# mayataka/idocp

Hardware: AMD Instinct MI355X
Metric: SQP iterations/sec (whole node) (higher is better)
Workload: dtype f64; 1 GPU; ANYmal OCPSolver N=100 T=5.05 FP64, trotting contact sequence (1 lift + 9 impulse events, 120 stages incl. impulse / aux / lift stages, switching constraints; BASELINE.json configs[2]); batch=1024 independent OCP instances per GPU, replicas across GPUs; horizon=100, batch_per_gpu=1024, parallelism=replicas x1

## Files before the change

idocp_amd/csrc/dev_rnea_tangent.hpp:

```cpp
#ifndef IDOCP_DEV_RNEA_TANGENT_HPP_
#define IDOCP_DEV_RNEA_TANGENT_HPP_

#include <hip/hip_runtime.h>

#include "dev_rbd.hpp"
#include "ocp_device.hpp"

namespace idocp_dev {

namespace rt {
struct V3 { double x, y, z; };
__device__ __forceinline__ V3 v3(double x, double y, double z) { V3 r; r.x = x; r.y = y; r.z = z; return r; }
__device__ __forceinline__ V3 ld3(const double* p) { return v3(p[0], p[1], p[2]); }
__device__ __forceinline__ void st3(double* p, V3 a) { p[0] = a.x; p[1] = a.y; p[2] = a.z; }
__device__ __forceinline__ V3 operator+(V3 a, V3 b) { return v3(a.x + b.x, a.y + b.y, a.z + b.z); }
__device__ __forceinline__ V3 operator-(V3 a, V3 b) { return v3(a.x - b.x, a.y - b.y, a.z - b.z); }
__device__ __forceinline__ V3 operator*(double s, V3 a) { return v3(s * a.x, s * a.y, s * a.z); }
__device__ __forceinline__ V3 cross(V3 a, V3 b) { return v3(a.y * b.z - a.z * b.y, a.z * b.x - a.x * b.z, a.x * b.y - a.y * b.x); }
__device__ __forceinline__ double dot(V3 a, V3 b) { return a.x * b.x + a.y * b.y + a.z * b.z; }
__device__ __forceinline__ V3 mul(const double* R, V3 a) {
  return v3(R[0] * a.x + R[1] * a.y + R[2] * a.z, R[3] * a.x + R[4] * a.y + R[5] * a.z, R[6] * a.x + R[7] * a.y + R[8] * a.z);
}
__device__ __forceinline__ V3 mulT(const double* R, V3 a) {
  return v3(R[0] * a.x + R[3] * a.y + R[6] * a.z, R[1] * a.x + R[4] * a.y + R[7] * a.z, R[2] * a.x + R[5] * a.y + R[8] * a.z);
// ... 130 lines not shown
  double* didc; int ldd;
  double* mm;
  double* jm; int ldj;
  double* idc;
};

template <typename D>
__device__ __forceinline__ void rneaSetup(const DevModel* __restrict__ m, const OcpProblem* __restrict__ P, const OcpNode* __restrict__ nd,
                                          int tid, double* sc) {
  using S = RneaScratch<D>;
  using namespace rt;
  constexpr int NL = D::NL, LJ = D::LJ, NJL = NL * LJ;
  if (tid >= 128 && tid < 128 + NJL) {
    const int t = tid - 128, ji = 1 + t;
    double* jr = sc + S::JOINTS + t * S::JREC;
    st3(jr + S::J_U, ld3(m->axis[ji])); st3(jr + S::J_P, ld3(m->p[ji]));
    jr[S::J_MASS] = m->mass[ji]; st3(jr + S::J_MC, ld3(m->mc[ji]));
#pragma unroll
    for (int e = 0; e < 6; ++e) jr[S::J_IO + e] = m->Io[ji][e];
  } else if (tid >= 192 && tid < 192 + NL) {
    const int leg = tid - 192;
    double* fr = sc + S::FEET + leg * S::FREC;
#pragma unroll
    for (int e = 0; e < 9; ++e) fr[S::F_RC + e] = P->contact_R[leg][e];
    st3(fr + S::F_PC, ld3(P->contact_p[leg]));
    fr[S::F_ACT] = nd->active[leg] ? 1.0 : 0.0;
    fr[S::F_ROW] = (double)nd->row_of[leg];
  } else if (tid == 192 + NL) {
    double* br = sc + S::BASE;
    br[S::B_MASS] = m->mass[0]; st3(br + S::B_MC, ld3(m->mc[0]));
#pragma unroll
    for (int e = 0; e < 6; ++e) br[S::B_IO + e] = m->Io[0][e];
  }
}

template <typename D, int NT>
struct RneaNominalCopy {
  using S = RneaScratch<D>;
  typedef double d2 __attribute__((ext_vector_type(2)));
  static constexpr int PER = (S::C_ALL + NT - 1) / NT;
  d2 r[PER];
  __device__ __forceinline__ void fetch(const double* __restrict__ nom, int tid) {
#pragma unroll
    for (int t = 0; t < PER; ++t) {
      const int c = tid + NT * t;
      r[t] = *reinterpret_cast<const d2*>(nom + 2 * (c < S::C_ALL ? c : 0));
    }
  }
  __device__ __forceinline__ void store(int tid, double* sc, double* idc) const {
#pragma unroll
    for (int t = 0; t < PER; ++t) {
      const int c = tid + NT * t;
      if (c < S::C_BN) *reinterpret_cast<d2*>(sc + S::pieceDst(c)) = r[t];
      else if (c < S::C_ALL) *reinterpret_cast<d2*>(idc + 2 * (c - S::C_BN)) = r[t];
    }
  }
};

template <typename D, bool XYY = false, bool IMPULSE = false>
__device__ __forceinline__ void rneaTangentItem(double gz, double wv, int item, double* sc, const RneaOut& out) {
  using S = RneaScratch<D>;
  using namespace rt;
  constexpr int LJ = D::LJ, NV = D::NV;
  const int leg = item / S::IPL, j0 = item - leg * S::IPL;
  const bool base_seed = j0 < 18;
  const int kind = base_seed ? j0 / 6 : (j0 - 18) / LJ;
  const int k = base_seed ? j0 - 6 * kind : 6 + leg * LJ + (j0 - 18 - LJ * kind);
  double* __restrict__ colp = (kind < 2) ? out.didc + (long)out.ldd * (kind * NV + k) : out.mm + NV * k;
  double* __restrict__ colc = (kind < 2) ? colp + NV : out.jm + (long)out.ldj * k;
  const double* br = sc + S::BASE;
  auto e3 = [](int i) { return v3(i == 0 ? 1.0 : 0.0, i == 1 ? 1.0 : 0.0, i == 2 ? 1.0 : 0.0); };
  const V3 zero = v3(0, 0, 0);
  V3 dz = (kind == 0 && k >= 3 && k < 6) ? cross(ld3(br + S::B_Z), e3(k - 3)) : zero;
  V3 dv = (kind == 1 && k < 3) ? e3(k) : zero, dw = (kind == 1 && k >= 3 && k < 6) ? e3(k - 3) : zero;
  V3 dbl = ((kind == 2 && k < 3) ? e3(k) : zero) - gz * dz, dbw = (kind == 2 && k >= 3 && k < 6) ? e3(k - 3) : zero;
  if (leg == 0 && base_seed) {
    V3 dhl, dhn, df, dn;
    const V3 mc = ld3(br + S::B_MC);
    inertia(br[S::B_MASS], mc, br + S::B_IO, dbl, dbw, df, dn);
    double* o = sc + S::BOWN + 6 * j0;
    if constexpr (IMPULSE) {
      st3(o, df); st3(o + 3, dn);
    } else {
      const V3 w0 = ld3(br + S::B_W), v0 = ld3(br + S::B_V), hl0 = ld3(br + S::B_HL), hn0 = ld3(br + S::B_HN);
      inertia(br[S::B_MASS], mc, br + S::B_IO, dv, dw, dhl, dhn);
      st3(o, df + cross(dw, hl0) + cross(w0, dhl));
      st3(o + 3, dn + cross(dw, hn0) + cross(w0, dhn) + cross(dv, hl0) + cross(v0, dhl));
    }
  }
  double tau[LJ];
#pragma unroll
  for (int j = 0; j < LJ; ++j) tau[j] = 0.0;
  V3 baseFl = zero, baseFn = zero;
  const double* jleg = sc + S::JOINTS + leg * LJ * S::JREC;
  forEachLegJointUnrolled<XYY, true, LJ>([&](auto tag, auto jc) {
    constexpr int AX = decltype(tag)::value, j = decltype(jc)::value;
    const int dof = 6 + leg * LJ + j;
    const double* jr = jleg + j * S::JREC;
    const bool mine = (k == dof);
    const double sq = (mine && kind == 0) ? 1.0 : 0.0, sv = (mine && kind == 1) ? 1.0 : 0.0, sa = (mine && kind == 2) ? 1.0 : 0.0;
    const JointFrame<AX> F(jr, S::J_R, S::J_U);
    {
      const V3 p = ld3(jr + S::J_P);
      const V3 wj = ld3(jr + S::J_W), vj = ld3(jr + S::J_VC);
      const V3 dwc = F.mulT(dw) - F.crossUk(ld3(jr + S::J_WC), sq);
      const V3 dvc = F.mulT(dv + cross(dw, p)) - F.crossUk(vj, sq);
      const V3 dbwc = F.mulT(dbw) - F.crossUk(ld3(jr + S::J_BWC), sq);
      const V3 dblc = F.mulT(dbl + cross(dbw, p)) - F.crossUk(ld3(jr + S::J_BLC), sq);
      dz = F.mulT(dz) - F.crossUk(ld3(jr + S::J_ZC), sq);
      dw = dwc + F.timesU(sv); dv = dvc;
      if constexpr (IMPULSE) {
        dbw = dbwc + F.timesU(sa); dbl = dblc;
      } else if constexpr (AX < 0) {
        const V3 vJ = ld3(jr + S::J_VJ), dvJ = F.timesU(sv);
        dbw = dbwc + F.timesU(sa) + cross(dw, vJ) + cross(wj, dvJ);
        dbl = dblc + cross(dv, vJ) + cross(vj, dvJ);
      } else {
        const double qd = jr[S::J_VJ + (AX < 0 ? 0 : AX)];
        dbw = dbwc + F.timesU(sa) + F.crossKU(dw, qd) + F.crossKU(wj, sv);
        dbl = dblc + F.crossKU(dv, qd) + F.crossKU(vj, sv);
      }
    }
    pin(dw); pin(dv); pin(dbw); pin(dbl); pin(dz);
    phaseFence();
    V3 Fl, Fn;
    {
      if constexpr (IMPULSE) {
        inertia(jr[S::J_MASS], ld3(jr + S::J_MC), jr + S::J_IO, dbl, dbw, Fl, Fn);
      } else {
        V3 dhl, dhn;
        {
          const V3 mc = ld3(jr + S::J_MC);
          inertia(jr[S::J_MASS], mc, jr + S::J_IO, dv, dw, dhl, dhn);
          inertia(jr[S::J_MASS], mc, jr + S::J_IO, dbl, dbw, Fl, Fn);
        }
        pin(dhl); pin(dhn); pin(Fl); pin(Fn);
        phaseFence();
        const V3 wj = ld3(jr + S::J_W), vj = ld3(jr + S::J_VC), hl = ld3(jr + S::J_HL), hn = ld3(jr + S::J_HN);
        Fl = Fl + cross(dw, hl) + cross(wj, dhl);
        Fn = Fn + cross(dw, hn) + cross(wj, dhn) + cross(dv, hl) + cross(vj, dhl);
      }
    }
    pin(Fl); pin(Fn);
    phaseFence();
    auto hop = [&](auto jjc) {
      constexpr int jj = decltype(jjc)::value;
      const double* jq = jleg + jj * S::JREC;
      const LegFrame<XYY, jj> G(jq, S::J_R, S::J_U);
      tau[jj] += G.dotU(Fn);
      if constexpr (jj == j) {
        Fl = Fl + G.crossUk(ld3(jq + S::J_FL), sq);
        Fn = Fn + G.crossUk(ld3(jq + S::J_FN), sq);
      }
      const V3 Rf = G.mul(Fl);
      Fn = G.mul(Fn) + cross(ld3(jq + S::J_P), Rf);
      Fl = Rf;
    };
    downFrom<j>(hop);
    baseFl = baseFl + Fl; baseFn = baseFn + Fn;
    pin(baseFl); pin(baseFn);
#pragma unroll
    for (int t = 0; t <= j; ++t) pin(tau[t]);
  });
  phaseFence();
  const double* fr = sc + S::FEET + leg * S::FREC;
  if (fr[S::F_ACT] != 0.0) {
    const double* Rc = fr + S::F_RC;
    const V3 pc = ld3(fr + S::F_PC);
    const V3 dal = dbl + gz * dz;
    const V3 dfv = XYY ? dv + cross(dw, pc) : mulT(Rc, dv + cross(dw, pc));
    if constexpr (IMPULSE) {
      st3(colc + (int)fr[S::F_ROW], dfv);
    } else {
      const V3 dfw = XYY ? dw : mulT(Rc, dw), dfa = XYY ? dal + cross(dbw, pc) : mulT(Rc, dal + cross(dbw, pc));
      const V3 dc = dfa + cross(ld3(fr + S::F_FW), dfv) + cross(ld3(fr + S::F_FV), dfw) + wv * dfv;
      st3(colc + (int)fr[S::F_ROW], dc);
    }
  }
#pragma unroll
  for (int j = 0; j < LJ; ++j) colp[6 + leg * LJ + j] = tau[j];
  double* o = sc + S::BT + 6 * item;
  st3(o, baseFl); st3(o + 3, baseFn);
}

template <typename D, bool XYY = false>
__device__ __forceinline__ void rneaTangentItemUndo(double gz, double wv, int item, double* sc, const RneaOut& out) {
  using S = RneaScratch<D>;
  using namespace rt;
  constexpr int LJ = D::LJ, NV = D::NV;
  const int leg = item / S::IPL, j0 = item - leg * S::IPL;
  const bool base_seed = j0 < 18;
  const int kind = base_seed ? j0 / 6 : (j0 - 18) / LJ;
  const int k = base_seed ? j0 - 6 * kind : 6 + leg * LJ + (j0 - 18 - LJ * kind);
  double* __restrict__ colp = (kind < 2) ? out.didc + (long)out.ldd * (kind * NV + k) : out.mm + NV * k;
  double* __restrict__ colc = (kind < 2) ? colp + NV : out.jm + (long)out.ldj * k;
  const double* br = sc + S::BASE;
  auto e3 = [](int i) { return v3(i == 0 ? 1.0 : 0.0, i == 1 ? 1.0 : 0.0, i == 2 ? 1.0 : 0.0); };
  const V3 zero = v3(0, 0, 0);
  V3 dz = (kind == 0 && k >= 3 && k < 6) ? cross(ld3(br + S::B_Z), e3(k - 3)) : zero;
  V3 dv = (kind == 1 && k < 3) ? e3(k) : zero, dw = (kind == 1 && k >= 3 && k < 6) ? e3(k - 3) : zero;
  V3 dbl = ((kind == 2 && k < 3) ? e3(k) : zero) - gz * dz, dbw = (kind == 2 && k >= 3 && k < 6) ? e3(k - 3) : zero;
  if (leg == 0 && base_seed) {
    V3 dhl, dhn, df, dn;
    const V3 mc = ld3(br + S::B_MC), w0 = ld3(br + S::B_W), v0 = ld3(br + S::B_V), hl0 = ld3(br + S::B_HL), hn0 = ld3(br + S::B_HN);
    inertia(br[S::B_MASS], mc, br + S::B_IO, dv, dw, dhl, dhn);
    inertia(br[S::B_MASS], mc, br + S::B_IO, dbl, dbw, df, dn);
    double* o = sc + S::BOWN + 6 * j0;
    st3(o, df + cross(dw, hl0) + cross(w0, dhl));
    st3(o + 3, dn + cross(dw, hn0) + cross(w0, dhn) + cross(dv, hl0) + cross(v0, dhl));
  }
  forEachLegJoint<XYY, true, LJ>([&](auto tag, int j) {
    constexpr int AX = decltype(tag)::value;
    const int dof = 6 + leg * LJ + j;
    const double* jr = sc + S::JOINTS + (leg * LJ + j) * S::JREC;
    const bool mine = (k == dof);
    const double sq = (mine && kind == 0) ? 1.0 : 0.0, sv = (mine && kind == 1) ? 1.0 : 0.0, sa = (mine && kind == 2) ? 1.0 : 0.0;
    const JointFrame<AX> F(jr, S::J_R, S::J_U);
    const V3 p = ld3(jr + S::J_P);
    const double qd = AX < 0 ? 0.0 : jr[S::J_VJ + (AX < 0 ? 0 : AX)];
    const V3 dwc = F.mulT(dw) - F.crossUk(ld3(jr + S::J_WC), sq);
    const V3 dvc = F.mulT(dv + cross(dw, p)) - F.crossUk(ld3(jr + S::J_VC), sq);
    const V3 dbwc = F.mulT(dbw) - F.crossUk(ld3(jr + S::J_BWC), sq);
    const V3 dblc = F.mulT(dbl + cross(dbw, p)) - F.crossUk(ld3(jr + S::J_BLC), sq);
    dz = F.mulT(dz) - F.crossUk(ld3(jr + S::J_ZC), sq);
    dw = dwc + F.timesU(sv); dv = dvc;
    if constexpr (AX < 0) {
      const V3 vJ = ld3(jr + S::J_VJ), dvJ = F.timesU(sv);
      dbw = dbwc + F.timesU(sa) + cross(dw, vJ) + cross(ld3(jr + S::J_W), dvJ);
      dbl = dblc + cross(dv, vJ) + cross(ld3(jr + S::J_VC), dvJ);
    } else {
      dbw = dbwc + F.timesU(sa) + F.crossKU(dw, qd) + F.crossKU(ld3(jr + S::J_W), sv);
      dbl = dblc + F.crossKU(dv, qd) + F.crossKU(ld3(jr + S::J_VC), sv);
    }
  });
  const double* fr = sc + S::FEET + leg * S::FREC;
  if (fr[S::F_ACT] != 0.0) {
    const double* Rc = fr + S::F_RC;
    const V3 pc = ld3(fr + S::F_PC);
    const V3 dal = dbl + gz * dz;
    const V3 dfv = XYY ? dv + cross(dw, pc) : mulT(Rc, dv + cross(dw, pc)), dfw = XYY ? dw : mulT(Rc, dw),
             dfa = XYY ? dal + cross(dbw, pc) : mulT(Rc, dal + cross(dbw, pc));
    const V3 dc = dfa + cross(ld3(fr + S::F_FW), dfv) + cross(ld3(fr + S::F_FV), dfw) + wv * dfv;
    st3(colc + (int)fr[S::F_ROW], dc);
  }
  V3 dFl = zero, dFn = zero;
  forEachLegJoint<XYY, false, LJ>([&](auto tag, int j) {
    constexpr int AX = decltype(tag)::value;
    const int dof = 6 + leg * LJ + j;
    const double* jr = sc + S::JOINTS + (leg * LJ + j) * S::JREC;
    const bool mine = (k == dof);
    const double sq = (mine && kind == 0) ? 1.0 : 0.0, sv = (mine && kind == 1) ? 1.0 : 0.0, sa = (mine && kind == 2) ? 1.0 : 0.0;
    const JointFrame<AX> F(jr, S::J_R, S::J_U);
    const V3 p = ld3(jr + S::J_P), mc = ld3(jr + S::J_MC);
    const V3 wj = ld3(jr + S::J_W), vj = ld3(jr + S::J_VC), hl = ld3(jr + S::J_HL), hn = ld3(jr + S::J_HN);
    V3 dhl, dhn, df, dn;
    inertia(jr[S::J_MASS], mc, jr + S::J_IO, dv, dw, dhl, dhn);
    inertia(jr[S::J_MASS], mc, jr + S::J_IO, dbl, dbw, df, dn);
    dFl = dFl + df + cross(dw, hl) + cross(wj, dhl);
    dFn = dFn + dn + cross(dw, hn) + cross(wj, dhn) + cross(dv, hl) + cross(vj, dhl);
    colp[dof] = F.dotU(dFn);
    const V3 dRf = F.mul(dFl + F.crossUk(ld3(jr + S::J_FL), sq));
    dFn = F.mul(dFn + F.crossUk(ld3(jr + S::J_FN), sq)) + cross(p, dRf);
    dFl = dRf;
    if (j > 0) {
      V3 dbwc, dblc;
// ... 168 lines not shown
```

idocp_amd/csrc/ocp_condense_kernel.hip:

```cpp
#include <hip/hip_runtime.h>

#include <cstdlib>

#include "dev_dense.hpp"
#include "dev_lie.hpp"
#include "dev_rnea_tangent.hpp"
#include "ocp_device.hpp"
#include "ocp_launch.hpp"

namespace idocp_dev {

#ifdef IDOCP_K5_TILES16
#define K5_TILE_PAIR mfmaTilePairTN
#else
#define K5_TILE_PAIR mfmaTilePairTN4
#endif

__device__ __forceinline__ double ocpLimit(const OcpProblem* __restrict__ P, int comp, int r) {
  switch (comp) {
    case 0: return P->q_min[r];
    case 1: return P->q_max[r];
    case 2: return -P->v_max[r];
    case 3: return P->v_max[r];
    case 4: return -P->u_max[r];
    case 8: return P->a_min[r];
    case 9: return P->a_max[r];
    default: return P->u_max[r];
  }
}
__device__ __forceinline__ bool ocpRowValid(const OcpProblem* __restrict__ P, int comp, int level, bool impulse) {
  if (impulse) return comp == 6 && P->use_impulse_friction_cone != 0;
  if (comp < 2) return P->use_q_limits && level >= 2;
  if (comp < 4) return P->use_v_limits && level >= 1;
  if (comp < 6) return P->use_u_limits != 0;
  if (comp == 8) return P->use_a_lower != 0;
  if (comp == 9) return P->use_a_upper != 0;
  return comp == 6 && P->use_friction_cone != 0;
}

template <typename D, int SFP = D::NF>
struct CondenseSmem {
  using L = OcpLayout<D>;
  static constexpr int NV = D::NV, NX = D::NX, NF = SFP, NVF = D::NV + SFP + (((D::NV + SFP) % 8 == 0) ? 2 : 0), NU = D::NU;
  static constexpr bool SEP_MINV = SFP <= 6;
  static constexpr int DIDC = 0, MM = DIDC + NVF * (NX + 1), JM = MM + NV * NV,
                       IDC = JM + ((NF * NV > NVF * NV - NV * NV) ? NF * NV : NVF * NV - NV * NV),
                       MJ = IDC + 32,
                       MJD = MJ + NVF * NVF,
                       QFF = (MJD + NVF * (NX + 1) > MJ + RneaScratch<D>::TOTAL) ? MJD + NVF * (NX + 1) : MJ + RneaScratch<D>::TOTAL, TMP = QFF + NF * NF,
                       QAFQV = DIDC, QAFU = MM, ERR = MJ;
  static constexpr int SOLS = TMP, SOLN = SOLS + L::SOL, SLK = SOLN + L::SOL, DUL = SLK + L::CON, TMP_EARLY = DUL + L::CON - TMP;
  static constexpr int BL = TMP, SM = BL + NF * NV, TMP_LATE = SM + NF * NF - TMP;
  static constexpr int VEC = TMP + (TMP_EARLY > TMP_LATE ? TMP_EARLY : TMP_LATE);
  static_assert(NVF * NV <= IDC - MM, "Qafu_full must fit in the M / J blocks");
  static_assert(512 <= NVF * NVF, "ERR (two accumulators per thread in the MERIT variant) aliases MJ");
  static constexpr int LQ = VEC, LV = LQ + NV, LA = LV + NV, LF = LA + NV, LU = LF + NF, LUP = LU + NU, FQ = LUP + 6, FV = FQ + NV,
                       LAF = FV + NV, TLA = LAF + 32, QAA = TLA + 32,
                       BM = QAA + NV,
                       LIEB = BM + 32, JQ = LIEB + L::Z_JQ, QDIFF = LIEB + L::Z_QDIFF, FQQ = LIEB + L::Z_FQQ, FQ6 = LIEB + L::Z_FQ6,
                       FQQI = LIEB + L::Z_FQQI, FQQP = LIEB + L::Z_FQQP, FQQPI = LIEB + L::Z_FQQPI,
                       HQD = LIEB + 196, HVD = HQD + NV, HUD = HVD + NV, QB6 = HUD + NU,
                       MINV = SEP_MINV ? QB6 + 36 + 2 : MM,
                       WSM = QB6 + 36 + 2 + (SEP_MINV ? NV * NV : 0),
                       TOTAL = WSM + (SEP_MINV ? 0 : NF * NF);
  static_assert(SOLS % 2 == 0 && LIEB % 2 == 0 && IDC % 2 == 0 && MJ % 2 == 0, "16-byte pieces");
};

__device__ __forceinline__ void blockLdsBarrier() {
  __builtin_amdgcn_fence(__ATOMIC_RELEASE, "workgroup", "local");
  __builtin_amdgcn_s_barrier();
  __builtin_amdgcn_fence(__ATOMIC_ACQUIRE, "workgroup", "local");
}

template <typename D, bool RESIDUAL, int DIMF, bool BWD = false, bool MERIT = false, bool XYY = false, bool EVENTS = false>
__global__ __launch_bounds__(256, 4) void ocp_condense_kernel(OcpBuffers B, const double* __restrict__ q0, const double* __restrict__ v0 = nullptr,
                                                              const int* __restrict__ plist = nullptr, int nlist = 0) {
  using L = OcpLayout<D>;
  using S = CondenseSmem<D, (DIMF > 0) ? DIMF : (DIMF == 0 ? D::NF / 2 : D::NF)>;
  constexpr int NV = D::NV, NQ = D::NQ, NX = D::NX, NF = D::NF, NVF = D::NVF, NU = D::NU, NC = D::NC;
  constexpr int SF = (DIMF > 0) ? DIMF : (DIMF == 0 ? NF / 2 : NF), SVF = S::NVF, RVF = NV + SF;
  extern __shared__ __attribute__((aligned(16))) double sm[];
  __shared__ int s_ok, s_c1, s_ba, s_gt, s_m;
  const OcpProblem* __restrict__ P = B.prob;
  const int M = B.M;
  int tid = threadIdx.x;
  tid = (((tid >> 6) + (int)(blockIdx.x & 3)) & 3) * 64 + (tid & 63);
  constexpr int nt = 256;
  const int per = plist ? nlist : M;
  auto stage = [&](const long unit) {
  const long b = unit / per;
  const int pos = plist ? plist[unit - b * per] : (int)(unit - b * per);
  const OcpNode* __restrict__ nd = B.nodes + pos;
  const bool terminal = (pos == M - 1);
  if (BWD && terminal) {
    if (MERIT && threadIdx.x < 2) B.merit_stage[(b * B.NS + nd->slot) * 4 + threadIdx.x] = 0.0;
    return;
  }
  const bool last = BWD && P->has_terminal && (pos == M - 2);
  constexpr bool PLAIN = (DIMF >= 0) && !EVENTS;
  const bool impulse = PLAIN ? false : (nd->kind == 1);
  if (BWD && impulse) return;
  const int sw_dimi = PLAIN ? 0 : nd->sw_dimi;
  int c_act[NC], c_row[NC];
#pragma unroll
  for (int c = 0; c < NC; ++c) { c_act[c] = nd->active[c]; c_row[c] = nd->row_of[c]; }
  const int i = nd->level;
  const double dt = nd->dt;
  const double dtq = nd->dtq;
  const int dimf = (DIMF >= 0) ? DIMF : nd->dimf, dimvf = NV + dimf;
  const int dimfd = (DIMF == 0) ? 1 : dimf;
  const long rec = b * B.NS + nd->slot;
  const double* __restrict__ s_g = B.sol + rec * L::SOL;
  const double* __restrict__ sn_g = B.sol + (b * B.NS + (terminal ? nd->slot : nd->next)) * L::SOL;
  const double* s = &sm[S::SOLS];
  const double* sn = &sm[S::SOLN];
  const double* q = s + L::S_Q;
  const double* __restrict__ qref = B.q_ref + (long)pos * NQ;
  const long su = rec;
#ifdef IDOCP_K5_STAMPS
  const bool stamp = (!RESIDUAL) && tid == 0 && unit == (long)(gridDim.x / 2 + 7) && B.prof != nullptr && DIMF == B.prof_dimf;
#define STAMP(k) do { if (stamp) B.prof[k] = wall_clock64(); } while (0)
  const bool stampw = (!RESIDUAL) && (tid & 63) == 0 && unit == (long)(gridDim.x / 2 + 7) && B.prof != nullptr && DIMF == B.prof_dimf;
#define STAMPW(k) do { if (stampw) B.prof[32 + 8 * (tid >> 6) + (k)] = wall_clock64(); } while (0)
#else
#define STAMP(k) do { } while (0)
#define STAMPW(k) do { } while (0)
#endif
  STAMP(0);
  double* kk = B.kkt + rec * L::KKT;
  double* ee = B.exp + rec * L::EXP;
  const double* __restrict__ w_q = impulse ? P->qi_weight : P->q_weight;
  const double* __restrict__ w_v = impulse ? P->vi_weight : P->v_weight;
  const double* __restrict__ w_a = impulse ? P->dvi_weight : P->a_weight;

  using RS = RneaScratch<D>;
  using RI = RneaItems<D>;
  static_assert(S::QFF - S::MJ >= RS::TOTAL, "the RNEA scratch lives in MJ .. MJD (dead until stage 3)");
  static_assert(S::MJ % 2 == 0 && S::IDC % 2 == 0, "16-byte pieces of the nominal record");
  static_assert(RI::NQV <= 64 && RI::NA <= 64, "one wavefront per item list");
  constexpr int NPRE = (2 * L::SOL + 2 * L::CON + nt - 1) / nt;
  static_assert(S::SOLN == S::SOLS + L::SOL && S::SLK == S::SOLN + L::SOL && S::DUL == S::SLK + L::CON, "the fetched records are contiguous in LDS");
  const int wave = tid >> 6, lane = tid & 63;
  double* const sc = &sm[S::MJ];
  RneaOut out;
  out.didc = &sm[S::DIDC]; out.ldd = SVF; out.mm = &sm[S::MM]; out.jm = &sm[S::JM]; out.ldj = SF; out.idc = &sm[S::IDC];
  {
    double pre[NPRE], prez[7];
    RneaNominalCopy<D, nt> nomc;
    const bool has_nom = !terminal;
    if (has_nom) nomc.fetch(B.nom + rec * L::NOM, tid);
#pragma unroll
    for (int t = 0; t < NPRE; ++t) {
      const int e = tid + nt * t;
      const double* src = e < L::SOL ? s_g + e : (e < 2 * L::SOL ? sn_g + (e - L::SOL) : (e < 2 * L::SOL + L::CON ? B.slack + su * L::CON + (e - 2 * L::SOL)
                                                                         : B.dual + su * L::CON + (e < 2 * L::SOL + 2 * L::CON ? e - 2 * L::SOL - L::CON : 0)));
      pre[t] = *src;
    }
    {
      const double* __restrict__ zz = B.lie + rec * L::LIE;
      if (tid < 36) { prez[0] = zz[L::Z_JQ + tid]; prez[1] = zz[L::Z_FQQ + tid]; prez[2] = zz[L::Z_FQQI + tid]; prez[3] = zz[L::Z_FQQP + tid]; prez[4] = zz[L::Z_FQQPI + tid]; }
      if (tid >= 64 && tid < 70) { prez[5] = zz[L::Z_QDIFF + tid - 64]; prez[6] = zz[L::Z_FQ6 + tid - 64]; }
    }
    STAMP(3);
    if (tid == 0) { s_ok = 1; s_c1 = 0; s_ba = 0; s_gt = 0; s_m = 0; }
    if (!terminal) {
      for (int e = tid; e < S::IDC - S::DIDC; e += nt) sm[S::DIDC + e] = 0.0;
      rneaSetup<D>(B.model, P, nd, tid, sc);
      nomc.store(tid, sc, &sm[S::IDC]);
    }
    for (int e = tid; e < SF * SF; e += nt) sm[S::QFF + e] = 0.0;
#pragma unroll
    for (int t = 0; t < NPRE; ++t) {
      const int e = tid + nt * t;
      if (e < 2 * L::SOL + 2 * L::CON) sm[S::SOLS + e] = pre[t];
    }
    if (tid < 36) { sm[S::JQ + tid] = prez[0]; sm[S::FQQ + tid] = prez[1]; sm[S::FQQI + tid] = prez[2]; sm[S::FQQP + tid] = prez[3]; sm[S::FQQPI + tid] = prez[4]; }
    if (tid >= 64 && tid < 70) { sm[S::QDIFF + tid - 64] = prez[5]; sm[S::FQ6 + tid - 64] = prez[6]; }
    STAMP(4);
  }
  blockLdsBarrier();
  STAMP(1);

  const double vref_on = nd->vref_on;
  const double v_ref0 = vref_on * P->v_ref[0];
  if (terminal) {
    if (tid < NV) {
      const int r = tid;
      double lq, lv;
      if (r < 6) {
        lq = 0.0;
        for (int m2 = 0; m2 < 6; ++m2) lq += sm[S::JQ + m2 + 6 * r] * P->qf_weight[m2] * sm[S::QDIFF + m2];
        double t1 = 0.0;
        for (int m2 = 0; m2 < 6; ++m2) t1 += sm[S::FQQP + m2 + 6 * r] * s[L::S_LMD + m2];
        lq += t1;
      } else {
        lq = P->qf_weight[r] * (q[r + 1] - qref[r + 1]) - s[L::S_LMD + r];
      }
      lv = P->vf_weight[r] * (s[L::S_V + r] - (r == 0 ? v_ref0 : vref_on * P->v_ref[r])) - s[L::S_GMM + r];
      if (B.ext) lq += B.ext[rec * L::EXT + L::X_LQ + r];
      if (MERIT) {
        const double qd = r < 6 ? sm[S::QDIFF + r] : q[r + 1] - qref[r + 1], dvr = s[L::S_V + r] - (r == 0 ? v_ref0 : vref_on * P->v_ref[r]);
        sm[S::ERR + tid] = 0.5 * (P->qf_weight[r] * qd * qd + P->vf_weight[r] * dvr * dvr);
      }
      else if (RESIDUAL) { sm[S::ERR + tid] = lq * lq + lv * lv; }
      else { kk[L::K_LX + r] = lq; kk[L::K_LX + NV + r] = lv; }
    } else if (RESIDUAL) {
      sm[S::ERR + tid] = 0.0;
    }
    if (RESIDUAL) {
      blockLdsBarrier();
      if (tid == 0) {
        double e = 0.0; for (int t = 0; t < nt; ++t) e += sm[S::ERR + t];
        if (MERIT) { B.merit_stage[rec * 4] = e + (B.ext ? B.ext[rec * L::EXT + L::X_COST] : 0.0); B.merit_stage[rec * 4 + 1] = 0.0; } else B.err_stage[rec] = e;
      }
      return;
    }
    for (int e = tid; e < NX * NX; e += nt) {
      const int c = e / NX, r = e - NX * c;
      double val = 0.0;
      if (r < 6 && c < 6) { for (int m2 = 0; m2 < 6; ++m2) val += sm[S::JQ + m2 + 6 * r] * P->qf_weight[m2] * sm[S::JQ + m2 + 6 * c]; }
      else if (r == c) val = (r < NV) ? P->qf_weight[r] : P->vf_weight[r - NV];
      if (r <= c) kk[L::K_QXX + L::xsym(r, c)] = val;
    }
    if (tid < 36) ee[L::E_FQQPI + tid] = sm[S::FQQPI + tid];
    return;
  }

  const double gz = B.model->gravity[2];
  const double bwv = 2.0 / P->baumgarte_time_step, bwp = 1.0 / (P->baumgarte_time_step * P->baumgarte_time_step);
  const double* slack = &sm[S::SLK];
  const double* dual = &sm[S::DUL];
  double err_local = 0.0, err_ipm = 0.0;
  double merit_cost = 0.0, merit_viol = 0.0;
  auto accelerationMultiplierTerm = [&](int lane_) {
    if (lane_ < NV) {
      double acc = dotAny(&sm[S::MM + NV * lane_], 1, s + L::S_BETA, 1, NV);
#pragma unroll
      for (int c = 0; c < NC; ++c) {
        if (!c_act[c]) continue;
        const double* jc = &sm[S::JM + c_row[c] + SF * lane_];
        acc += jc[0] * s[L::S_MU + 3 * c] + jc[1] * s[L::S_MU + 3 * c + 1] + jc[2] * s[L::S_MU + 3 * c + 2];
      }
      sm[S::TLA + lane_] = acc;
    }
  };
  if (wave == 0) {
    if (!MERIT && lane < RI::NQV) {
      if (!PLAIN && impulse) rneaTangentItem<D, XYY, true>(0.0, bwv, RI::qv(lane), sc, out);
      else rneaTangentItem<D, XYY, false>(gz, bwv, RI::qv(lane), sc, out);
    }
    STAMPW(0);
  } else if (wave == 1) {
    if (!MERIT) {
      {
        if (lane < RI::NA) rneaTangentItemA<D, XYY>(RI::a(lane), sc, out);
        waveLdsSync();
        rneaAssembleA<D>(lane, sc, out);
        waveLdsSync();
#ifdef IDOCP_K5_REP_AITEMS
        asm volatile("" ::: "memory");
        if (lane < RI::NA) rneaTangentItemA<D, XYY>(RI::a(lane), sc, out);
        waveLdsSync();
        rneaAssembleA<D>(lane, sc, out);
        waveLdsSync();
#endif
      }
      STAMPW(0);
      if (!RESIDUAL) {
        if constexpr (S::SEP_MINV) ldsFlagSet(&s_m, 1, lane);
        else { accelerationMultiplierTerm(lane); waveLdsSync(); }
        STAMPW(4);
#ifdef IDOCP_K5_STAMPS
        blockArrowInverse<6, D::NL, D::LJ>(&sm[S::MINV], NV, lane, &s_ok, stampw ? B.prof + 16 : nullptr, &s_ba, &s_gt, &sm[S::MM]);
#else
        blockArrowInverse<6, D::NL, D::LJ>(&sm[S::MINV], NV, lane, &s_ok, nullptr, &s_ba, &s_gt, &sm[S::MM]);
#endif
        STAMPW(1);
        STAMPW(3);
      }
    }
  } else if (tid < 128 + NV) {
    const int r = tid - 128;
    const double vr = s[L::S_V + r], ar = s[L::S_A + r];
    const double lmd = s[L::S_LMD + r], gmm = s[L::S_GMM + r], lmdn = sn[L::S_LMD + r], gmmn = sn[L::S_GMM + r];
    double lq, lv, la, hq = 0.0, hv, ha;
    const double* __restrict__ sp_g = (BWD && nd->prev >= 0) ? B.sol + (b * B.NS + nd->prev) * L::SOL : nullptr;
    const double qpr = !BWD ? 0.0 : (sp_g ? sp_g[L::S_Q + r + 1] : q0[b * NQ + r + 1]);
    const double vpr = !BWD ? 0.0 : (sp_g ? sp_g[L::S_V + r] : v0[b * NV + r]);
    double fq;
    if (r < 6) {
      lq = 0.0;
      for (int m2 = 0; m2 < 6; ++m2) lq += sm[S::JQ + m2 + 6 * r] * w_q[m2] * sm[S::QDIFF + m2];
      lq *= dt;
      double t1 = 0.0;
      for (int m2 = 0; m2 < 6; ++m2) t1 += sm[S::FQQ + m2 + 6 * r] * sn[L::S_LMD + m2] + sm[S::FQQP + m2 + 6 * r] * s[L::S_LMD + m2];
      lq += t1;
      fq = sm[S::FQ6 + r] + dtq * vr;
    } else {
      lq = dt * w_q[r] * (q[r + 1] - qref[r + 1]) + lmdn - lmd;
      hq = dt * w_q[r];
      fq = BWD ? (qpr - q[r + 1] + dtq * vr) : (q[r + 1] - sn[L::S_Q + r + 1] + dtq * vr);
    }
    sm[S::FQ + r] = fq;
    lv = dt * w_v[r] * (vr - (r == 0 ? v_ref0 : vref_on * P->v_ref[r])) + (BWD ? dtq * lmd : dtq * lmdn) + gmmn - gmm;
    la = dt * w_a[r] * ar + dt * (BWD ? gmm : gmmn);
    hv = dt * w_v[r];
    ha = dt * w_a[r];
    const double fv = BWD ? (vpr - vr + dt * ar) : (vr + dt * ar - sn[L::S_V + r]);
    sm[S::FV + r] = fv;
    if (MERIT) {
      const double qd = r < 6 ? sm[S::QDIFF + r] : q[r + 1] - qref[r + 1], dvr = vr - (r == 0 ? v_ref0 : vref_on * P->v_ref[r]);
      merit_cost += 0.5 * dt * (w_q[r] * qd * qd + w_v[r] * dvr * dvr + w_a[r] * ar * ar);
      merit_viol += fabs(fq) + fabs(fv);
    }
    if (last) {
      if (r < 6) {
        double tq = 0.0;
        for (int m2 = 0; m2 < 6; ++m2) tq += sm[S::JQ + m2 + 6 * r] * P->qf_weight[m2] * sm[S::QDIFF + m2];
        lq += tq;
      } else {
        lq += P->qf_weight[r] * (q[r + 1] - qref[r + 1]);
        hq += P->qf_weight[r];
      }
      lv += P->vf_weight[r] * (vr - (r == 0 ? v_ref0 : vref_on * P->v_ref[r]));
      hv += P->vf_weight[r];
    }
    if (r >= 6) {
      const int j = r - 6;
      for (int c = 0; c < 4; ++c) {
        if (!ocpRowValid(P, c, i, impulse)) continue;
        const double sgn = (c & 1) ? 1.0 : -1.0;
        const double x = (c < 2) ? q[r + 1] : vr;
        const double sl = slack[c * NU + j], du = dual[c * NU + j];
        const double res = sgn * (x - ocpLimit(P, c, j)) + sl, duality = sl * du - P->barrier;
        double g = sgn * dt * du, h = 0.0;
        if (MERIT) merit_viol += dt * fabs(res);
        if (RESIDUAL) err_ipm += res * res + duality * duality;
        else { const double isl = recipNewton(sl); g += sgn * dt * (du * res - duality) * isl; h = dt * du * isl; }
        if (c < 2) { lq += g; hq += h; } else { lv += g; hv += h; }
      }
      if (P->use_a_lower | P->use_a_upper) {
        for (int c = 8; c < 10; ++c) {
          if (!ocpRowValid(P, c, i, impulse)) continue;
          const double sgn = (c & 1) ? 1.0 : -1.0;
          const int row = L::C_ACC + (c - 8) * NU + j;
          const double sl = slack[row], du = dual[row];
          const double res = sgn * (ar - ocpLimit(P, c, j)) + sl, duality = sl * du - P->barrier;
          double g = sgn * dt * du, h = 0.0;
          if (MERIT) merit_viol += dt * fabs(res);
          if (RESIDUAL) err_ipm += res * res + duality * duality;
          else { const double isl = recipNewton(sl); g += sgn * dt * (du * res - duality) * isl; h = dt * du * isl; }
          la += g; ha += h;
        }
// ... 11 lines not shown
    sm[S::BM + r] = s[L::S_BETA + r];
    if (!RESIDUAL) { sm[S::HQD + r] = hq; sm[S::HVD + r] = hv; }
    else err_local += fq * fq + fv * fv;
  } else if (tid >= 128 + 32 && tid < 128 + 32 + NU) {
    const int j = tid - 128 - 32;
    const double u = s[L::S_U + j];
    double lu = dt * P->u_weight[j] * (u - P->u_ref[j]) - dt * s[L::S_BETA + 6 + j];
    double h = dt * P->u_weight[j];
    if (impulse) { lu = 0.0; h = 1.0; }
    if (MERIT && !impulse) merit_cost += 0.5 * dt * P->u_weight[j] * (u - P->u_ref[j]) * (u - P->u_ref[j]);
    for (int c = 4; c < 6; ++c) {
      if (!ocpRowValid(P, c, i, impulse)) continue;
      const double sgn = (c & 1) ? 1.0 : -1.0;
      const double sl = slack[c * NU + j], du = dual[c * NU + j];
      const double res = sgn * (u - ocpLimit(P, c, j)) + sl, duality = sl * du - P->barrier;
      if (MERIT) merit_viol += dt * fabs(res);
      lu += sgn * dt * du;
      if (RESIDUAL) err_ipm += res * res + duality * duality;
      else { const double isl = recipNewton(sl); lu += sgn * dt * (du * res - duality) * isl; h += dt * du * isl; }
    }
    sm[S::LU + j] = lu;
    if (!RESIDUAL) sm[S::HUD + j] = h;
    else err_local += lu * lu;
  } else if (tid >= 128 + 48 && tid < 128 + 48 + 6) {
    const int r = tid - 128 - 48;
    const double lup = impulse ? 0.0 : dt * s[L::S_NUP + r] - dt * s[L::S_BETA + r];
    sm[S::LUP + r] = lup;
    if (RESIDUAL) err_local += lup * lup;
  } else if (tid >= 192 && tid < 192 + NC) {
    const int c = tid - 192;
    if (nd->active[c]) {
      const int row = nd->row_of[c];
      double lf[3], f[3];
      for (int x = 0; x < 3; ++x) {
        f[x] = s[L::S_F + 3 * c + x];
        const double wf = impulse ? P->fi_weight[c][x] : P->f_weight[c][x], rf = impulse ? P->fi_ref[c][x] : P->f_ref[c][x];
        lf[x] = dt * wf * (f[x] - rf);
        if (MERIT) merit_cost += 0.5 * dt * wf * (f[x] - rf) * (f[x] - rf);
        if (!RESIDUAL) sm[S::QFF + (row + x) + SF * (row + x)] = dt * wf;
        sm[S::BM + NV + row + x] = s[L::S_MU + 3 * c + x];
      }
      if (ocpRowValid(P, 6, i, impulse)) {
        const int ck = impulse ? P->impulse_cone_kind : P->cone_kind, nr = coneRows(ck);
        double dd[5], Jr[5][3];
        for (int r = 0; r < 5; ++r) {
          if (r >= nr) { dd[r] = 0.0; Jr[r][0] = Jr[r][1] = Jr[r][2] = 0.0; continue; }
          const int idx = L::C_FRIC + 5 * c + r;
          const double sl = slack[idx], du = dual[idx];
          const double g = coneRow(ck, P->mu, r, f, Jr[r]);
          const double res = g + sl, duality = sl * du - P->barrier;
          double coef = du;
          const double isl = recipNewton(sl);
          if (MERIT) merit_viol += dt * fabs(res);
          if (RESIDUAL) err_ipm += res * res + duality * duality;
          else coef += (du * res - duality) * isl;
          dd[r] = du * isl;
          for (int x = 0; x < 3; ++x) lf[x] += dt * Jr[r][x] * coef;
        }
        if (!RESIDUAL) {
          for (int x = 0; x < 3; ++x) for (int y = 0; y < 3; ++y) {
            double acc = 0.0;
            for (int r = 0; r < 5; ++r) acc += Jr[r][x] * dd[r] * Jr[r][y];
            sm[S::QFF + (row + x) + SF * (row + y)] += dt * acc;
          }
        }
      }
      for (int x = 0; x < 3; ++x) sm[S::LF + row + x] = lf[x];
    }
  } else if (!RESIDUAL && tid >= 192 + 8 && tid < 192 + 8 + 36) {
    const int e = tid - 192 - 8, c = e / 6, r = e - 6 * c;
    double acc = 0.0;
    for (int m2 = 0; m2 < 6; ++m2) acc += sm[S::JQ + m2 + 6 * r] * w_q[m2] * sm[S::JQ + m2 + 6 * c];
    double accf = 0.0;
    if (last) for (int m2 = 0; m2 < 6; ++m2) accf += sm[S::JQ + m2 + 6 * r] * P->qf_weight[m2] * sm[S::JQ + m2 + 6 * c];
    sm[S::QB6 + e] = dt * acc + accf;
    double fqq = 0.0;
    for (int m2 = 0; m2 < 6; ++m2) fqq += sm[S::FQQI + r + 6 * m2] * sm[(BWD ? S::FQQP : S::FQQ) + m2 + 6 * c];
    kk[L::K_FQQ + e] = BWD ? fqq : -fqq;
    kk[L::K_FQV + e] = (BWD ? dtq : -dtq) * sm[S::FQQI + e];
    ee[L::E_FQQPI + e] = sm[(BWD ? S::FQQI : S::FQQPI) + e];
  }
  if (wave >= 2) STAMPW(0);
  if (wave >= 2 && !MERIT && !RESIDUAL) {
    if constexpr (S::SEP_MINV) {
      if (wave == 3) { ldsFlagWait(&s_m, 1, lane); accelerationMultiplierTerm(lane); }
    }
    __builtin_amdgcn_fence(__ATOMIC_RELEASE, "workgroup");
    __builtin_amdgcn_wave_barrier();
    if (lane == 0) __hip_atomic_fetch_add(&s_c1, 1, __ATOMIC_RELAXED, __HIP_MEMORY_SCOPE_WORKGROUP);
    constexpr int NJ = D::NL * D::LJ, LJ = D::LJ;
    constexpr int GG = S::SM + SF * SF, TT = GG + SF * 6;
    static_assert(TT + SF * NJ <= S::VEC, "G and Jl D^-1 fit behind BL, SM");
    ldsFlagWait(&s_c1, 2, lane);
    ldsFlagWait(&s_ba, 1, lane);
    if (wave == 2) {
      for (int e = lane; e < dimf * 6; e += 64) {
        const int c = e / dimfd, r = e - c * dimfd;
        double acc = sm[S::JM + r + SF * c];
#pragma unroll
        for (int m = 0; m < NJ; ++m) acc -= sm[S::JM + r + SF * (6 + m)] * sm[S::MINV + (6 + m) + NV * c];
        sm[GG + r + SF * c] = acc;
      }
      for (int e = lane; e < dimf * NJ; e += 64) {
        const int c = e / dimfd, r = e - c * dimfd, o = 6 + (c / LJ) * LJ;
        double acc = 0.0;
#pragma unroll
        for (int m = 0; m < LJ; ++m) acc += sm[S::JM + r + SF * (o + m)] * sm[S::MINV + (o + m) + NV * (6 + c)];
        sm[TT + r + SF * c] = acc;
      }
      waveLdsSync();
      ldsFlagSet(&s_gt, 1, lane);
      ldsFlagWait(&s_ba, 2, lane);
      for (int e = lane; e < dimf * 6; e += 64) {
        const int c = e / dimfd, r = e - c * dimfd;
        double acc = 0.0;
#pragma unroll
        for (int m = 0; m < 6; ++m) acc += sm[GG + r + SF * m] * sm[S::MINV + m + NV * c];
        sm[S::BL + r + SF * c] = acc;
      }
      waveLdsSync();
      for (int e = lane; e < dimf * dimf; e += 64) {
        const int c = e / dimfd, r = e - c * dimfd;
        double acc = 0.0;
#pragma unroll
        for (int m = 0; m < 6; ++m) acc += sm[S::BL + r + SF * m] * sm[GG + c + SF * m];
#pragma unroll
        for (int m = 0; m < NJ; ++m) acc += sm[TT + r + SF * m] * sm[S::JM + c + SF * (6 + m)];
        sm[S::SM + r + SF * c] = acc;
      }
      waveLdsSync();
      if (dimf > 0) {
        constexpr int WW = (TT + SF * NJ + SF * SF <= S::VEC) ? TT + SF * NJ : S::WSM;
        static_assert(WW != S::WSM || !S::SEP_MINV, "the narrow layouts keep W behind G and Jl D^-1");
        spdInverseCholDpp<SF>(&sm[S::SM], SF, dimf, lane, &s_ok, &sm[WW], SF);
      }
    } else {
      ldsFlagWait(&s_gt, 1, lane);
      ldsFlagWait(&s_ba, 3, lane);
      for (int e = lane; e < dimf * NJ; e += 64) {
        const int c = e / dimfd, r = e - c * dimfd;
        double acc = sm[TT + r + SF * c];
#pragma unroll
        for (int m = 0; m < 6; ++m) acc += sm[GG + r + SF * m] * sm[S::MINV + m + NV * (6 + c)];
        sm[S::BL + r + SF * (6 + c)] = acc;
      }
    }
    STAMPW(3);
  }
  blockLdsBarrier();
  STAMP(2);
  if (MERIT) {
    rneaAssembleNominal<D>(tid, sc, out);
    blockLdsBarrier();
    if (!impulse && tid >= 6 && tid < NV && nd->has_u) sm[S::IDC + tid] -= s_g[L::S_U + tid - 6];
    blockLdsBarrier();
    if (tid < dimvf) merit_viol += dt * fabs(sm[S::IDC + tid]);
    if (sw_dimi > 0 && tid >= 200 && tid < 200 + sw_dimi) merit_viol += fabs(B.swc[rec * L::SWC + L::W_P + tid - 200]);
    blockLdsBarrier();
    sm[S::ERR + tid] = merit_cost; sm[S::ERR + nt + tid] = merit_viol;
    blockLdsBarrier();
    if (tid < 2) {
      double e = 0.0;
      for (int t = 0; t < nt; ++t) e += sm[S::ERR + nt * tid + t];
      if (B.ext) e += B.ext[rec * L::EXT + (tid == 1 ? L::X_VIOL : L::X_COST)];
      B.merit_stage[rec * 4 + tid] = e;
    }
    return;
  }
  STAMP(5);
  asm volatile("" : "+v"(tid) :: "memory");
  if (RESIDUAL) {
    rneaAssembleQV<D>(bwp, tid, nt, sc, out);
    blockLdsBarrier();
    if (!impulse && tid >= 6 && tid < NV && nd->has_u) sm[S::IDC + tid] -= s_g[L::S_U + tid - 6];
    blockLdsBarrier();
    if (tid >= 128 && tid < 128 + NV) {
      const int r = tid - 128;
      const double dq = dotAny(&sm[S::DIDC + SVF * r], 1, &sm[S::BM], 1, dimvf);
      const double dv = dotAny(&sm[S::DIDC + SVF * (NV + r)], 1, &sm[S::BM], 1, dimvf);
      const double da = dotAny(&sm[S::MM + NV * r], 1, &sm[S::BM], 1, NV) + dotAny(&sm[S::JM + SF * r], 1, &sm[S::BM + NV], 1, dimf);
      const double lq = sm[S::LQ + r] + dt * dq, lv = sm[S::LV + r] + dt * dv, la = sm[S::LA + r] + dt * da;
      const double idr = sm[S::IDC + r];
      err_local += lq * lq + lv * lv + la * la + dt * dt * idr * idr;
    } else if (tid >= 192 && tid < 192 + NC) {
      const int c = tid - 192;
      if (nd->active[c]) {
        const int row = nd->row_of[c];
        for (int x = 0; x < 3; ++x) {
          double jb = 0.0;
          for (int col = 0; col < NV; ++col) jb += sm[S::JM + (row + x) + SF * col] * sm[S::BM + col];
          const double lf = sm[S::LF + row + x] - dt * jb;
          const double cr = sm[S::IDC + NV + row + x];
          err_local += lf * lf + dt * dt * cr * cr;
        }
      }
    }
    if (sw_dimi > 0 && tid >= 200 && tid < 200 + sw_dimi) {
      const double pr = B.swc[rec * L::SWC + L::W_P + tid - 200];
      err_local += pr * pr;
    }
    blockLdsBarrier();
    sm[S::ERR + tid] = err_local + (BWD ? 1.0 : dt * dt) * err_ipm;
    blockLdsBarrier();
    if (tid == 0) {
      double e = 0.0;
      for (int t = 0; t < nt; ++t) e += sm[S::ERR + t];
      if (B.ext) e += (BWD ? 1.0 : dt * dt) * B.ext[rec * L::EXT + L::X_ERR];
      B.err_stage[rec] = e;
    }
    return;
  }
  constexpr bool EARLY_MJ = (SVF * SVF <= RS::FEET);
  auto assembleTR = [&]() {
    for (int e = tid; e < dimf * NV; e += nt) {
      const int c = e / NV, r = e - c * NV;
      const double tr = dotAny(&sm[S::BL + SF * r], 1, &sm[S::SM + SF * c], 1, dimf);
// ... 421 lines not shown
```

Before: 216,300 SQP iterations/s.

## Shrink condense-kernel LDS and registers to fit five workgroups per CU

Repacks the condense kernel's LDS layout for narrow contact dimensions. It stages only the used prefixes of the solution, slack and dual records, aliases several scratch vectors into dead regions, and drops the separate M^-1 copy together with its extra wave handoff. Launch bounds are raised to five workgroups per CU when the stage fits under the per-CU LDS ceiling. The RNEA tangent item also splits its cross-product chains with phase fences and accumulates tau and the base wrench directly in LDS instead of in registers, to cut register pressure. The trade-off is extra LDS traffic and serialization in exchange for higher occupancy.

After: 214,900 SQP iterations/s. About the same (-0.7%).

```diff
diff --git a/idocp_amd/csrc/dev_rnea_tangent.hpp b/idocp_amd/csrc/dev_rnea_tangent.hpp
--- a/idocp_amd/csrc/dev_rnea_tangent.hpp
+++ b/idocp_amd/csrc/dev_rnea_tangent.hpp
@@ -236,16 +236,30 @@
     if constexpr (IMPULSE) {
       st3(o, df); st3(o + 3, dn);
     } else {
-      const V3 w0 = ld3(br + S::B_W), v0 = ld3(br + S::B_V), hl0 = ld3(br + S::B_HL), hn0 = ld3(br + S::B_HN);
       inertia(br[S::B_MASS], mc, br + S::B_IO, dv, dw, dhl, dhn);
-      st3(o, df + cross(dw, hl0) + cross(w0, dhl));
-      st3(o + 3, dn + cross(dw, hn0) + cross(w0, dhn) + cross(dv, hl0) + cross(v0, dhl));
-    }
-  }
-  double tau[LJ];
-#pragma unroll
-  for (int j = 0; j < LJ; ++j) tau[j] = 0.0;
-  V3 baseFl = zero, baseFn = zero;
+      pin(dhl); pin(dhn); pin(df); pin(dn);
+      phaseFence();
+      {
+        const V3 w0 = ld3(br + S::B_W), hl0 = ld3(br + S::B_HL);
+        st3(o, df + cross(dw, hl0) + cross(w0, dhl));
+      }
+      phaseFence();
+      {
+        const V3 w0 = ld3(br + S::B_W), hn0 = ld3(br + S::B_HN);
+        dn = dn + cross(dw, hn0) + cross(w0, dhn);
+        pin(dn);
+      }
+      phaseFence();
+      {
+        const V3 v0 = ld3(br + S::B_V), hl0 = ld3(br + S::B_HL);
+        st3(o + 3, dn + cross(dv, hl0) + cross(v0, dhl));
+      }
+    }
+    phaseFence();
+  }
+  double* const taup = colp + 6 + leg * LJ;
+  double* const btp = sc + S::BT + 6 * item;
+  st3(btp, zero); st3(btp + 3, zero);
   const double* jleg = sc + S::JOINTS + leg * LJ * S::JREC;
   forEachLegJointUnrolled<XYY, true, LJ>([&](auto tag, auto jc) {
     constexpr int AX = decltype(tag)::value, j = decltype(jc)::value;
@@ -255,14 +269,20 @@
     const double sq = (mine && kind == 0) ? 1.0 : 0.0, sv = (mine && kind == 1) ? 1.0 : 0.0, sa = (mine && kind == 2) ? 1.0 : 0.0;
     const JointFrame<AX> F(jr, S::J_R, S::J_U);
     {
+      dz = F.mulT(dz) - F.crossUk(ld3(jr + S::J_ZC), sq);
+      pin(dz);
+      phaseFence();
       const V3 p = ld3(jr + S::J_P);
-      const V3 wj = ld3(jr + S::J_W), vj = ld3(jr + S::J_VC);
-      const V3 dwc = F.mulT(dw) - F.crossUk(ld3(jr + S::J_WC), sq);
-      const V3 dvc = F.mulT(dv + cross(dw, p)) - F.crossUk(vj, sq);
+      {
+        const V3 dwc = F.mulT(dw) - F.crossUk(ld3(jr + S::J_WC), sq);
+        const V3 dvc = F.mulT(dv + cross(dw, p)) - F.crossUk(ld3(jr + S::J_VC), sq);
+        dw = dwc + F.timesU(sv); dv = dvc;
+      }
+      pin(dw); pin(dv);
+      phaseFence();
       const V3 dbwc = F.mulT(dbw) - F.crossUk(ld3(jr + S::J_BWC), sq);
       const V3 dblc = F.mulT(dbl + cross(dbw, p)) - F.crossUk(ld3(jr + S::J_BLC), sq);
-      dz = F.mulT(dz) - F.crossUk(ld3(jr + S::J_ZC), sq);
-      dw = dwc + F.timesU(sv); dv = dvc;
+      const V3 wj = ld3(jr + S::J_W), vj = ld3(jr + S::J_VC);
       if constexpr (IMPULSE) {
         dbw = dbwc + F.timesU(sa); dbl = dblc;
       } else if constexpr (AX < 0) {
@@ -290,9 +310,22 @@
         }
         pin(dhl); pin(dhn); pin(Fl); pin(Fn);
         phaseFence();
-        const V3 wj = ld3(jr + S::J_W), vj = ld3(jr + S::J_VC), hl = ld3(jr + S::J_HL), hn = ld3(jr + S::J_HN);
-        Fl = Fl + cross(dw, hl) + cross(wj, dhl);
-        Fn = Fn + cross(dw, hn) + cross(wj, dhn) + cross(dv, hl) + cross(vj, dhl);
+        {
+          const V3 wj = ld3(jr + S::J_W), hl = ld3(jr + S::J_HL);
+          Fl = Fl + cross(dw, hl) + cross(wj, dhl);
+          pin(Fl);
+        }
+        phaseFence();
+        {
+          const V3 wj = ld3(jr + S::J_W), hn = ld3(jr + S::J_HN);
+          Fn = Fn + cross(dw, hn) + cross(wj, dhn);
+          pin(Fn);
+        }
+        phaseFence();
+        {
+          const V3 vj = ld3(jr + S::J_VC), hl = ld3(jr + S::J_HL);
+          Fn = Fn + cross(dv, hl) + cross(vj, dhl);
+        }
       }
     }
     pin(Fl); pin(Fn);
@@ -301,7 +334,7 @@
       constexpr int jj = decltype(jjc)::value;
       const double* jq = jleg + jj * S::JREC;
       const LegFrame<XYY, jj> G(jq, S::J_R, S::J_U);
-      tau[jj] += G.dotU(Fn);
+      taup[jj] = taup[jj] + G.dotU(Fn);
       if constexpr (jj == j) {
         Fl = Fl + G.crossUk(ld3(jq + S::J_FL), sq);
         Fn = Fn + G.crossUk(ld3(jq + S::J_FN), sq);
@@ -311,10 +344,7 @@
       Fl = Rf;
     };
     downFrom<j>(hop);
-    baseFl = baseFl + Fl; baseFn = baseFn + Fn;
-    pin(baseFl); pin(baseFn);
-#pragma unroll
-    for (int t = 0; t <= j; ++t) pin(tau[t]);
+    st3(btp, ld3(btp) + Fl); st3(btp + 3, ld3(btp + 3) + Fn);
   });
   phaseFence();
   const double* fr = sc + S::FEET + leg * S::FREC;
@@ -331,10 +361,6 @@
       st3(colc + (int)fr[S::F_ROW], dc);
     }
   }
-#pragma unroll
-  for (int j = 0; j < LJ; ++j) colp[6 + leg * LJ + j] = tau[j];
-  double* o = sc + S::BT + 6 * item;
-  st3(o, baseFl); st3(o + 3, baseFn);
 }
 
 template <typename D, bool XYY = false>
diff --git a/idocp_amd/csrc/ocp_condense_kernel.hip b/idocp_amd/csrc/ocp_condense_kernel.hip
--- a/idocp_amd/csrc/ocp_condense_kernel.hip
+++ b/idocp_amd/csrc/ocp_condense_kernel.hip
@@ -42,29 +42,42 @@
 struct CondenseSmem {
   using L = OcpLayout<D>;
   static constexpr int NV = D::NV, NX = D::NX, NF = SFP, NVF = D::NV + SFP + (((D::NV + SFP) % 8 == 0) ? 2 : 0), NU = D::NU;
-  static constexpr bool SEP_MINV = SFP <= 6;
+  static constexpr bool NARROW = SFP <= 6;
   static constexpr int DIDC = 0, MM = DIDC + NVF * (NX + 1), JM = MM + NV * NV,
                        IDC = JM + ((NF * NV > NVF * NV - NV * NV) ? NF * NV : NVF * NV - NV * NV),
-                       MJ = IDC + 32,
+                       MJ = IDC + (NARROW ? L::NVF : 32),
                        MJD = MJ + NVF * NVF,
                        QFF = (MJD + NVF * (NX + 1) > MJ + RneaScratch<D>::TOTAL) ? MJD + NVF * (NX + 1) : MJ + RneaScratch<D>::TOTAL, TMP = QFF + NF * NF,
                        QAFQV = DIDC, QAFU = MM, ERR = MJ;
-  static constexpr int SOLS = TMP, SOLN = SOLS + L::SOL, SLK = SOLN + L::SOL, DUL = SLK + L::CON, TMP_EARLY = DUL + L::CON - TMP;
+  static constexpr int SOLS_LEN = NARROW ? (L::S_XI + L::NF + 1) / 2 * 2 : L::SOL, SOLN_LEN = NARROW ? (L::S_A + 1) / 2 * 2 : L::SOL,
+                       CON_LEN = NARROW ? (L::C_CD + 1) / 2 * 2 : L::CON, STAGED = SOLS_LEN + SOLN_LEN + 2 * CON_LEN;
+  static constexpr int SOLS = TMP, SOLN = SOLS + SOLS_LEN, SLK = SOLN + SOLN_LEN, DUL = SLK + CON_LEN, TMP_EARLY = DUL + CON_LEN - TMP;
   static constexpr int BL = TMP, SM = BL + NF * NV, TMP_LATE = SM + NF * NF - TMP;
   static constexpr int VEC = TMP + (TMP_EARLY > TMP_LATE ? TMP_EARLY : TMP_LATE);
+  static_assert(SOLS_LEN <= L::SOL && SOLN_LEN <= L::SOL && CON_LEN <= L::CON, "the staged pieces lie inside their records");
   static_assert(NVF * NV <= IDC - MM, "Qafu_full must fit in the M / J blocks");
   static_assert(512 <= NVF * NVF, "ERR (two accumulators per thread in the MERIT variant) aliases MJ");
+  static constexpr int JGAP = JM + NF * NV;
+  static_assert(!NARROW || (IDC - JGAP >= NV + NF && MJ - IDC >= NV + NF), "bm behind J, laf over [ID; C]");
   static constexpr int LQ = VEC, LV = LQ + NV, LA = LV + NV, LF = LA + NV, LU = LF + NF, LUP = LU + NU, FQ = LUP + 6, FV = FQ + NV,
-                       LAF = FV + NV, TLA = LAF + 32, QAA = TLA + 32,
-                       BM = QAA + NV,
-                       LIEB = BM + 32, JQ = LIEB + L::Z_JQ, QDIFF = LIEB + L::Z_QDIFF, FQQ = LIEB + L::Z_FQQ, FQ6 = LIEB + L::Z_FQ6,
+                       LAF = NARROW ? IDC : FV + NV, TLA = NARROW ? FV + NV : LAF + 32,
+                       QAA = TLA + (NARROW ? NV : 32),
+                       BM = NARROW ? JGAP : QAA + NV,
+                       LIEB = NARROW ? QAA + NV : BM + 32, JQ = LIEB + L::Z_JQ, QDIFF = LIEB + L::Z_QDIFF, FQQ = LIEB + L::Z_FQQ, FQ6 = LIEB + L::Z_FQ6,
                        FQQI = LIEB + L::Z_FQQI, FQQP = LIEB + L::Z_FQQP, FQQPI = LIEB + L::Z_FQQPI,
                        HQD = LIEB + 196, HVD = HQD + NV, HUD = HVD + NV, QB6 = HUD + NU,
-                       MINV = SEP_MINV ? QB6 + 36 + 2 : MM,
-                       WSM = QB6 + 36 + 2 + (SEP_MINV ? NV * NV : 0),
-                       TOTAL = WSM + (SEP_MINV ? 0 : NF * NF);
+                       MINV = MM,
+                       WSM = QB6 + 36 + 2,
+                       TOTAL = NARROW ? QB6 + 36 : WSM + NF * NF;
   static_assert(SOLS % 2 == 0 && LIEB % 2 == 0 && IDC % 2 == 0 && MJ % 2 == 0, "16-byte pieces");
 };
+
+constexpr int K5_LDS_PER_CU = 160 * 1024, K5_LDS_GRANULE = 512, K5_STATIC_LDS = 32;
+constexpr int K5_LDS_CEILING = K5_LDS_PER_CU / 5 / K5_LDS_GRANULE * K5_LDS_GRANULE - K5_STATIC_LDS;
+template <typename D, int DIMF, bool RESIDUAL, bool XYY>
+constexpr int k5WorkgroupsPerCU() {
+  return (DIMF > 0 && CondenseSmem<D, (DIMF > 0) ? DIMF : D::NF>::NARROW && !RESIDUAL && XYY) ? 5 : 4;
+}
 
 __device__ __forceinline__ void blockLdsBarrier() {
   __builtin_amdgcn_fence(__ATOMIC_RELEASE, "workgroup", "local");
@@ -73,14 +86,16 @@
 }
 
 template <typename D, bool RESIDUAL, int DIMF, bool BWD = false, bool MERIT = false, bool XYY = false, bool EVENTS = false>
-__global__ __launch_bounds__(256, 4) void ocp_condense_kernel(OcpBuffers B, const double* __restrict__ q0, const double* __restrict__ v0 = nullptr,
+__global__ __launch_bounds__(256, (k5WorkgroupsPerCU<D, DIMF, RESIDUAL, XYY>())) void ocp_condense_kernel(OcpBuffers B, const double* __restrict__ q0, const double* __restrict__ v0 = nullptr,
                                                               const int* __restrict__ plist = nullptr, int nlist = 0) {
   using L = OcpLayout<D>;
   using S = CondenseSmem<D, (DIMF > 0) ? DIMF : (DIMF == 0 ? D::NF / 2 : D::NF)>;
   constexpr int NV = D::NV, NQ = D::NQ, NX = D::NX, NF = D::NF, NVF = D::NVF, NU = D::NU, NC = D::NC;
   constexpr int SF = (DIMF > 0) ? DIMF : (DIMF == 0 ? NF / 2 : NF), SVF = S::NVF, RVF = NV + SF;
   extern __shared__ __attribute__((aligned(16))) double sm[];
-  __shared__ int s_ok, s_c1, s_ba, s_gt, s_m;
+  static_assert(k5WorkgroupsPerCU<D, DIMF, RESIDUAL, XYY>() < 5 || S::TOTAL * (int)sizeof(double) <= K5_LDS_CEILING,
+                "five resident workgroups: the stage's LDS plus the status words within a fifth of the CU's, in whole granules");
+  __shared__ int s_ok, s_c1, s_ba, s_gt;
   const OcpProblem* __restrict__ P = B.prob;
   const int M = B.M;
   int tid = threadIdx.x;
@@ -138,8 +153,10 @@
   static_assert(S::QFF - S::MJ >= RS::TOTAL, "the RNEA scratch lives in MJ .. MJD (dead until stage 3)");
   static_assert(S::MJ % 2 == 0 && S::IDC % 2 == 0, "16-byte pieces of the nominal record");
   static_assert(RI::NQV <= 64 && RI::NA <= 64, "one wavefront per item list");
-  constexpr int NPRE = (2 * L::SOL + 2 * L::CON + nt - 1) / nt;
-  static_assert(S::SOLN == S::SOLS + L::SOL && S::SLK == S::SOLN + L::SOL && S::DUL == S::SLK + L::CON, "the fetched records are contiguous in LDS");
+  constexpr int NPRE = (S::STAGED + nt - 1) / nt;
+  constexpr int E_SN = S::SOLS_LEN, E_SLK = E_SN + S::SOLN_LEN, E_DUL = E_SLK + S::CON_LEN;
+  static_assert(S::SOLN == S::SOLS + E_SN && S::SLK == S::SOLS + E_SLK && S::DUL == S::SOLS + E_DUL && S::STAGED == E_DUL + S::CON_LEN,
+                "the fetched records are contiguous in LDS");
   const int wave = tid >> 6, lane = tid & 63;
   double* const sc = &sm[S::MJ];
   RneaOut out;
@@ -152,8 +169,8 @@
 #pragma unroll
     for (int t = 0; t < NPRE; ++t) {
       const int e = tid + nt * t;
-      const double* src = e < L::SOL ? s_g + e : (e < 2 * L::SOL ? sn_g + (e - L::SOL) : (e < 2 * L::SOL + L::CON ? B.slack + su * L::CON + (e - 2 * L::SOL)
-                                                                         : B.dual + su * L::CON + (e < 2 * L::SOL + 2 * L::CON ? e - 2 * L::SOL - L::CON : 0)));
+      const double* src = e < E_SN ? s_g + e : (e < E_SLK ? sn_g + (e - E_SN) : (e < E_DUL ? B.slack + su * L::CON + (e - E_SLK)
+                                                                         : B.dual + su * L::CON + (e < S::STAGED ? e - E_DUL : 0)));
       pre[t] = *src;
     }
     {
@@ -162,7 +179,7 @@
       if (tid >= 64 && tid < 70) { prez[5] = zz[L::Z_QDIFF + tid - 64]; prez[6] = zz[L::Z_FQ6 + tid - 64]; }
     }
     STAMP(3);
-    if (tid == 0) { s_ok = 1; s_c1 = 0; s_ba = 0; s_gt = 0; s_m = 0; }
+    if (tid == 0) { s_ok = 1; s_c1 = 0; s_ba = 0; s_gt = 0; }
     if (!terminal) {
       for (int e = tid; e < S::IDC - S::DIDC; e += nt) sm[S::DIDC + e] = 0.0;
       rneaSetup<D>(B.model, P, nd, tid, sc);
@@ -172,7 +189,7 @@
 #pragma unroll
     for (int t = 0; t < NPRE; ++t) {
       const int e = tid + nt * t;
-      if (e < 2 * L::SOL + 2 * L::CON) sm[S::SOLS + e] = pre[t];
+      if (e < S::STAGED) sm[S::SOLS + e] = pre[t];
     }
     if (tid < 36) { sm[S::JQ + tid] = prez[0]; sm[S::FQQ + tid] = prez[1]; sm[S::FQQI + tid] = prez[2]; sm[S::FQQP + tid] = prez[3]; sm[S::FQQPI + tid] = prez[4]; }
     if (tid >= 64 && tid < 70) { sm[S::QDIFF + tid - 64] = prez[5]; sm[S::FQ6 + tid - 64] = prez[6]; }
@@ -267,8 +284,7 @@
       }
       STAMPW(0);
       if (!RESIDUAL) {
-        if constexpr (S::SEP_MINV) ldsFlagSet(&s_m, 1, lane);
-        else { accelerationMultiplierTerm(lane); waveLdsSync(); }
+        accelerationMultiplierTerm(lane); waveLdsSync();
         STAMPW(4);
 #ifdef IDOCP_K5_STAMPS
         blockArrowInverse<6, D::NL, D::LJ>(&sm[S::MINV], NV, lane, &s_ok, stampw ? B.prof + 16 : nullptr, &s_ba, &s_gt, &sm[S::MM]);
@@ -446,9 +462,6 @@
   }
   if (wave >= 2) STAMPW(0);
   if (wave >= 2 && !MERIT && !RESIDUAL) {
-    if constexpr (S::SEP_MINV) {
-      if (wave == 3) { ldsFlagWait(&s_m, 1, lane); accelerationMultiplierTerm(lane); }
-    }
     __builtin_amdgcn_fence(__ATOMIC_RELEASE, "workgroup");
     __builtin_amdgcn_wave_barrier();
     if (lane == 0) __hip_atomic_fetch_add(&s_c1, 1, __ATOMIC_RELAXED, __HIP_MEMORY_SCOPE_WORKGROUP);
@@ -495,7 +508,7 @@
       waveLdsSync();
       if (dimf > 0) {
         constexpr int WW = (TT + SF * NJ + SF * SF <= S::VEC) ? TT + SF * NJ : S::WSM;
-        static_assert(WW != S::WSM || !S::SEP_MINV, "the narrow layouts keep W behind G and Jl D^-1");
+        static_assert(WW != S::WSM || !S::NARROW, "the narrow layouts keep W behind G and Jl D^-1");
         spdInverseCholDpp<SF>(&sm[S::SM], SF, dimf, lane, &s_ok, &sm[WW], SF);
       }
     } else {
```
